# rageworx/libsrcnn

Hardware: AMD Instinct MI355X
Metric: megapixels/sec SRCNN Y-channel (2x upscale) (higher is better)
Workload: dtype f32

## Files before the change

### libsrcnn_amd/build.py

```python
import os
import subprocess
import sys

HERE = os.path.dirname(os.path.abspath(__file__))
CSRC = os.path.join(HERE, "csrc")
LIBDIR = os.path.join(HERE, "lib")
LIB = os.path.join(LIBDIR, "libsrcnn_amd.so")

SOURCES = ["srcnn_kernels.hip", "srcnn_fused_f16.hip", "srcnn_yuv_planes.hip", "srcnn_yuv_packed.hip", "srcnn_rgb.hip", "srcnn_rgb_window.hip", "srcnn_yuv_window.hip", "srcnn_yuv_packed_window.hip", "srcnn_window.hip", "srcnn_capi.cpp", "srcnn_frames.cpp", "srcnn_pipeline.cpp", "srcnn_comm.cpp", "dropin.cpp"]
DEPS = SOURCES + ["../../tools/srcnntest.cpp", "../../tools/srcnnyuv.cpp", "srcnn_kernels.h", "srcnn_yuv.h", "srcnn_rgb.h", "srcnn_window.h", "srcnn_frame_rules.h", "srcnn_frame_args.hpp", "srcnn_rect_source.hpp", "srcnn_pixel_io.h", "srcnn_colour_rules.h", "srcnn_window_tile.h", "srcnn_yuv_packed_fields.h", "srcnn_host.hpp", "srcnn_owned.hpp", "srcnn_settings.hpp", "srcnn_watchdog.hpp", "resample_table.hpp", "srcnn_weights.inc",
                  "../../include/srcnn_amd.h", "../../include/srcnn_amd_debug.h", "../../include/srcnn_amd_yuv.h", "../../include/srcnn_amd_yuv_ex.h", "../../include/srcnn_amd_yuv_packed.h", "../../include/srcnn_amd_rgb.h", "../../include/srcnn_amd_rect.h", "../../include/srcnn_amd_rgb_rect.h", "../../include/srcnn_amd_yuv_rect.h", "../../include/srcnn_amd_yuv_packed_rect.h",
                  "../../include/libsrcnn_dropin.h", "exports.map"]

FLAGS = ["--offload-arch=gfx950", "-O3", "-ffp-contract=off", "-fPIC", "-std=c++17",
         "-fvisibility=hidden", "-Wall", "-Wno-unused-result", "-Wno-unused-value", "-Wno-ignored-attributes", "-D__HIP_PLATFORM_AMD__"]


EXTRA_FLAGS = {"srcnn_fused_f16.hip": ["-fno-slp-vectorize"] + os.environ.get("SRCNN_FUSED_CFLAGS", "").split()}


def hipcc():
    for c in (os.environ.get("HIPCC"), "/opt/rocm/bin/hipcc", "hipcc"):
        if c and (os.path.isabs(c) and os.path.exists(c) or not os.path.isabs(c)):
            return c
    return "hipcc"


STAMP = os.path.join(LIBDIR, "build.sha256")


def source_digest():
    import hashlib
    h = hashlib.sha256()
    h.update(repr((FLAGS, sorted(EXTRA_FLAGS.items()))).encode())
    for d in sorted(set(DEPS)) + [os.path.abspath(__file__)]:
        path = d if os.path.isabs(d) else os.path.join(CSRC, d)
        h.update(os.path.basename(path).encode() + b"\0")
        with open(path, "rb") as f:
            h.update(f.read())
    return h.hexdigest()


def stale():
    if not all(os.path.exists(p) for p in (LIB, STAMP, os.path.join(LIBDIR, "libsrcnn.so"), os.path.join(LIBDIR, "libsrcnn.a"))):
        return True
    try:
        return open(STAMP).read().strip() != source_digest()
    except OSError:
        return True


def _region(src, start_pat, end_pat):
    import re
    m = re.search(start_pat, src)
    if not m:
        return None
    e = re.search(end_pat, src[m.end():])
    return src[m.start():m.end() + (e.start() if e else len(src) - m.end())]


def kernel_source_sha(name="k_conv12_mfma"):
    import hashlib
    import re
    src = open(os.path.join(CSRC, "srcnn_kernels.hip")).read()
    m = re.search(r"template <[^>]*>\s*__global__[^\n]*void %s\(" % re.escape(name), src)
    if not m:
        return None
    end = src.find("// ====", m.end())
    parts = [src[m.start():end if end > 0 else len(src)]]
    extra = []
    if name == "k_conv12_mfma":
        extra = [_region(src, r"constexpr int M_NW\b", r"\n// One tap-step"),
                 _region(src, r"__device__ __forceinline__ void rs_dma_dword\(", r"\n}\n"),
                 _region(src, r"void conv12_grid_info\(", r"\n}\n"),
                 _region(src, r"void launch_conv12_mfma\(", r"\n}\n"),
                 _region(open(os.path.join(CSRC, "srcnn_capi.cpp")).read(), r"void run_conv12\(", r"\n}\n")]
    elif name == "k_conv3":
        extra = [_region(src, r"constexpr int C3_TW\b", r"\ntemplate <bool STRICT"),
                 _region(src, r"__device__ __forceinline__ void rs_dma_dword\(", r"\n}\n"),
                 _region(src, r"void launch_conv3\(", r"\n}\n")]
    if any(e is None for e in extra):
        return None
    h = hashlib.sha256()
    for part in parts + extra:
        h.update(part.encode())
        h.update(b"\0")
    return h.hexdigest()


STRICT_DIR = os.path.join(LIBDIR, "strict")
STRICT_LIB = os.path.join(STRICT_DIR, "libsrcnn_amd.so")


def build_strict_only(force=False, verbose=True):
    import time
    stamp = os.path.join(STRICT_DIR, "build.sha256")
    digest = source_digest() + "-strict"
    if not force and os.path.exists(STRICT_LIB) and os.path.exists(stamp) and open(stamp).read().strip() == digest:
        return STRICT_LIB, None
    os.makedirs(STRICT_DIR, exist_ok=True)
    t0 = time.time()
    objs = []
    for src in SOURCES:
        if src == "srcnn_fused_f16.hip":
            continue
        obj = os.path.join(STRICT_DIR, os.path.splitext(src)[0] + ".o")
        cmd = [hipcc()] + FLAGS + ["-DSRCNN_STRICT_ONLY"] + ["-x", "hip", "-c", os.path.join(CSRC, src), "-o", obj]
        if verbose:
            print(" ".join(cmd), flush=True)
        subprocess.check_call(cmd)
        objs.append(obj)
    cmd = [hipcc(), "--offload-arch=gfx950", "-shared", "-fPIC"] + objs + ["-o", STRICT_LIB, "-ldl", "-Wl,-soname,libsrcnn_amd.so",
                                                                          "-Wl,--version-script=" + os.path.join(CSRC, "exports.map")]
    if verbose:
        print(" ".join(cmd), flush=True)
    subprocess.check_call(cmd)
    with open(stamp, "w") as f:
        f.write(digest + "\n")
    return STRICT_LIB, time.time() - t0


def build(force=False, verbose=True):
    if not force and not stale():
        return LIB
    os.makedirs(LIBDIR, exist_ok=True)
    objs = []
    for src in SOURCES:
        obj = os.path.join(LIBDIR, os.path.splitext(src)[0] + ".o")
        cmd = [hipcc()] + FLAGS + EXTRA_FLAGS.get(src, []) + ["-x", "hip", "-c", os.path.join(CSRC, src), "-o", obj]
        if verbose:
            print(" ".join(cmd), flush=True)
        subprocess.check_call(cmd)
# ... 38 lines not shown
```

### libsrcnn_amd/csrc/srcnn_capi.cpp

```cpp
#include <dlfcn.h>
#include <hip/hip_runtime.h>
#include <sys/prctl.h>
#include <sys/syscall.h>
#include <unistd.h>

#include <algorithm>
#include <cstdio>
#include <cstdlib>
#include <cstring>
#include <string>
#include <thread>

#include "resample_table.hpp"
#include <chrono>
#include <sys/auxv.h>
#include <unistd.h>

#include "../../include/srcnn_amd_rect.h"
#include "srcnn_frame_args.hpp"
#include "srcnn_host.hpp"
#include "srcnn_rect_source.hpp"
#include "srcnn_window.h"

namespace srcnn {
// ... 823 lines not shown
                        unsigned r0, unsigned r1, float* d_dst)
{
    return resample_src_rows(c, YSource::from_plane(d_in), sw, sh, dw, dh, filter, r0, r1, d_dst);
}

int check_plane(const void* in, unsigned w, unsigned h, const void* out)
{
    if (!in || !out || w == 0 || h == 0) return fail(SRCNN_E_ARG, "NULL pointer or zero dimension");
    if ((unsigned long long)w * h > 0x7fffffffULL) return fail(SRCNN_E_UNSUPPORTED, "plane too large");
    return SRCNN_OK;
}

int y_path_rows(Call& c, const YSource& src, unsigned w, unsigned h, unsigned dw, unsigned dh, int filter,
                unsigned r0, unsigned r1, float* d_out)
{
    if (r1 > dh || r0 >= r1) return fail(SRCNN_E_ARG, "row range [%u,%u) outside 0..%u", r0, r1, dh);
    if (dh > (1u << 20) || h > (1u << 20) || dw > 0x7fffffu || (r1 - r0) > 65535u * 16u)
        return fail(SRCNN_E_UNSUPPORTED, "output %ux%u too large", dw, dh);
    Workspace& ws = *c.ws;
    [[maybe_unused]] Ctx& cx = *c.cx;
    const unsigned ca = r0 >= 2 ? r0 - 2 : 0, cb = std::min(dh, r1 + 2);
    const unsigned ua = ca >= 4 ? ca - 4 : 0, ub = std::min(dh, cb + 4);
    int rc;
    if ((rc = ws.grow(ws.up, (size_t)dw * (ub - ua)))) return rc;
#ifndef SRCNN_STRICT_ONLY
    const bool fused = c.mode == SRCNN_MODE_FAST_F16;
    if (fused) {
        {
            StageTimer t(SRCNN_STAGE_RESAMPLE, c);
            if ((rc = resample_src_rows(c, src, w, h, dw, dh, filter, ua, ub, ws.up.data()))) return rc;
        }
        {
            StageTimer t(SRCNN_STAGE_CONV12, c);
            launch_fused_f16(ws.up.data(), (int)dw, (int)dh, (int)ua, (int)(ub - ua), d_out, (int)r0, (int)(r1 - r0), cx.fused_w.data(),
                             cx.num_cus, c.s);
        }
        HIP_TRY(hipGetLastError());
        return SRCNN_OK;
    }
#endif
    if ((rc = ws.grow(ws.c2, (size_t)C2N * dw * (cb - ca)))) return rc;
    TraceRange tr("srcnn y_path rows [%u,%u) of %ux%u", r0, r1, dw, dh);
    {
        StageTimer t(SRCNN_STAGE_RESAMPLE, c);
        if ((rc = resample_src_rows(c, src, w, h, dw, dh, filter, ua, ub, ws.up.data()))) return rc;
    }
    const size_t plane = (size_t)dw * (cb - ca);
    {
        StageTimer t(SRCNN_STAGE_CONV12, c);
        run_conv12(c, ws.up.data(), (int)dw, (int)dh, (int)ua, (int)(ub - ua), ws.c2.data(), plane, (int)ca, (int)(cb - ca));
    }
    {
        StageTimer t(SRCNN_STAGE_CONV3, c);
        launch_conv3(ws.c2.data(), plane, (int)dw, (int)dh, (int)ca, (int)(cb - ca), d_out, (int)r0, (int)(r1 - r0),
                     c.relax(), c.s);
    }
    if (const hipError_t e = hipGetLastError(); e != hipSuccess) {
        ws.queue_dirty = true;
        return fail(SRCNN_E_HIP, "y_path_rows: %s", hipGetErrorString(e));
    }
    return SRCNN_OK;
}

int y_path_source_rows(Call& c, unsigned h, unsigned dh, int filter, unsigned r0, unsigned r1, unsigned& lo, unsigned& hi)
{
    const unsigned ca = r0 >= 2 ? r0 - 2 : 0, cb = std::min(dh, r1 + 2);
    const unsigned ua = ca >= 4 ? ca - 4 : 0, ub = std::min(dh, cb + 4);
    if (h == dh) { lo = ua; hi = ub; return SRCNN_OK; }
    TableRef tv;
    int rc = get_table(c, filter, dh, h, tv);
    if (rc) return rc;
    tv->source_span(ua, ub, lo, hi);
    hi = std::min(hi, h);
    return SRCNN_OK;
}

unsigned budget_band_rows(unsigned dw)
{
    const size_t budget = G.ws_budget.load();
    const size_t row_bytes = (size_t)C2N * dw * sizeof(float);
    const size_t fit = budget / row_bytes;
    return (unsigned)std::min<size_t>(std::max<size_t>(16, fit > 4 ? fit - 4 : 1), 1u << 20);
}

std::vector<unsigned> plan_cuts(unsigned R0, unsigned R1, unsigned dw, unsigned dh, const double* frac, int nfrac, int grid, int tile_rows)
{
    const unsigned rows = R1 - R0;
    std::vector<unsigned> cuts{R0};
    const unsigned tiles_x = (dw + 63) / 64;
    unsigned a = R0;
    for (int i = 0; i < nfrac; ++i) {
        const unsigned want = std::max(32u, (unsigned)(rows * frac[i]));
        unsigned b = a + (want & ~15u);
        if (grid > 0 && tile_rows > 0) {
            const unsigned top = a >= 2 ? 2 : a;
            const unsigned t_want = (want + top + 2 + tile_rows - 1) / tile_rows;
            const unsigned t_lo = std::max(1u, (unsigned)(t_want * 0.7)), t_hi = std::max(t_lo, (unsigned)(t_want * 1.3));
            double best = -1.0;
            unsigned best_t = t_want;
            for (unsigned t = t_lo; t <= t_hi; ++t) {
                const unsigned long long tiles = (unsigned long long)t * tiles_x;
                const unsigned long long rounds = (tiles + grid - 1) / grid;
                const double fill = (double)tiles / (double)(rounds * grid);
                const double score = fill - 1e-4 * (t > t_want ? t - t_want : t_want - t);
                if (score > best) { best = score; best_t = t; }
            }
            if (best_t * tile_rows > top + 2) b = a + best_t * tile_rows - top - 2;
// ... 25 lines not shown
}

int y_path_frame(Call& c, const float* d_in, unsigned w, unsigned h, unsigned dw, unsigned dh, int filter, float* d_out)
{
    return y_path_range(c, d_in, w, h, dw, dh, filter, 0, dh, d_out);
}

namespace {

int y_path_rect_rows(Call& c, const float* d_in, size_t in_stride, unsigned in_x0, unsigned in_y0, unsigned w, unsigned h,
                     unsigned dw, unsigned dh, int filter, unsigned x0, unsigned x1, unsigned r0, unsigned r1, float* d_out,
                     size_t out_stride)
{
    Workspace& ws = *c.ws;
    [[maybe_unused]] Ctx& cx = *c.cx;
    const unsigned cax = x0 >= 2 ? x0 - 2 : 0, cbx = std::min(dw, x1 + 2);
    const unsigned uax = cax >= 4 ? cax - 4 : 0, ubx = std::min(dw, cbx + 4);
    const unsigned Ww = ubx - uax;
    const unsigned ca = r0 >= 2 ? r0 - 2 : 0, cb = std::min(dh, r1 + 2);
    const unsigned ua = ca >= 4 ? ca - 4 : 0, ub = std::min(dh, cb + 4);
    int rc;
    if ((rc = ws.grow(ws.up, (size_t)Ww * (ub - ua)))) return rc;
    if ((rc = ws.grow(ws.win, (size_t)Ww * (r1 - r0)))) return rc;
    const float* interior = ws.win.data() + (x0 - uax);
#ifndef SRCNN_STRICT_ONLY
    if (c.mode == SRCNN_MODE_FAST_F16) {
        {
            StageTimer t(SRCNN_STAGE_RESAMPLE, c);
            if ((rc = resample_window(c, d_in, in_stride, in_x0, in_y0, w, h, dw, dh, filter, uax, ubx, ua, ub, ws.up.data()))) return rc;
        }
        {
            StageTimer t(SRCNN_STAGE_CONV12, c);
            launch_fused_f16(ws.up.data(), (int)Ww, (int)dh, (int)ua, (int)(ub - ua), ws.win.data(), (int)r0, (int)(r1 - r0), cx.fused_w.data(),
                             cx.num_cus, c.s);
        }
        launch_window_copy(interior, Ww, d_out, out_stride, (int)(x1 - x0), (int)(r1 - r0), c.s);
        HIP_TRY(hipGetLastError());
        return SRCNN_OK;
    }
#endif
    if ((rc = ws.grow(ws.c2, (size_t)C2N * Ww * (cb - ca)))) return rc;
    TraceRange tr("srcnn y_path rect [%u,%u)x[%u,%u) of %ux%u", x0, x1, r0, r1, dw, dh);
    {
        StageTimer t(SRCNN_STAGE_RESAMPLE, c);
        if ((rc = resample_window(c, d_in, in_stride, in_x0, in_y0, w, h, dw, dh, filter, uax, ubx, ua, ub, ws.up.data()))) return rc;
    }
    const size_t plane = (size_t)Ww * (cb - ca);
    {
        StageTimer t(SRCNN_STAGE_CONV12, c);
        run_conv12(c, ws.up.data(), (int)Ww, (int)dh, (int)ua, (int)(ub - ua), ws.c2.data(), plane, (int)ca, (int)(cb - ca));
    }
    {
        StageTimer t(SRCNN_STAGE_CONV3, c);
        launch_conv3(ws.c2.data(), plane, (int)Ww, (int)dh, (int)ca, (int)(cb - ca), ws.win.data(), (int)r0, (int)(r1 - r0), c.relax(), c.s);
    }
    launch_window_copy(interior, Ww, d_out, out_stride, (int)(x1 - x0), (int)(r1 - r0), c.s);
    if (const hipError_t e = hipGetLastError(); e != hipSuccess) {
        ws.queue_dirty = true;
        return fail(SRCNN_E_HIP, "y_path_rect: %s", hipGetErrorString(e));
    }
    return SRCNN_OK;
}

}

int y_path_rect(Call& c, const float* d_in, size_t in_stride, unsigned in_x0, unsigned in_y0, unsigned w, unsigned h, unsigned dw,
                unsigned dh, int filter, unsigned x0, unsigned y0, unsigned x1, unsigned y1, float* d_out, size_t out_stride, bool whole_plane)
{
    if (x1 > dw || x0 >= x1 || y1 > dh || y0 >= y1) return fail(SRCNN_E_ARG, "rect [%u,%u)x[%u,%u) outside %ux%u", x0, x1, y0, y1, dw, dh);
    if (dh > (1u << 20) || h > (1u << 20) || dw > 0x7fffffu || (y1 - y0) > 65535u * 16u)
        return fail(SRCNN_E_UNSUPPORTED, "output %ux%u too large", dw, dh);
    if (x0 == 0 && x1 == dw && whole_plane && in_x0 == 0 && in_y0 == 0 && in_stride == w && out_stride == dw)
        return y_path_range(c, d_in, w, h, dw, dh, filter, y0, y1, d_out);
    const unsigned cax = x0 >= 2 ? x0 - 2 : 0, cbx = std::min(dw, x1 + 2);
    const unsigned Ww = std::min(dw, cbx + 4) - (cax >= 4 ? cax - 4 : 0);
    const size_t row_bytes = (size_t)C2N * Ww * sizeof(float);
    const bool no_planes = c.mode == SRCNN_MODE_FAST_F16;
    if (no_planes || row_bytes * ((size_t)(y1 - y0) + 4) <= G.ws_budget.load())
        return y_path_rect_rows(c, d_in, in_stride, in_x0, in_y0, w, h, dw, dh, filter, x0, x1, y0, y1, d_out, out_stride);
    const unsigned band = budget_band_rows(Ww);
    for (unsigned a = y0; a < y1; a += band) {
        const unsigned b = std::min(y1, a + band);
        int rc = y_path_rect_rows(c, d_in, in_stride, in_x0, in_y0, w, h, dw, dh, filter, x0, x1, a, b, d_out + (size_t)(a - y0) * out_stride, out_stride);
        if (rc) return rc;
    }
    return SRCNN_OK;
}

unsigned y_path_rect_band_rows(const Call& c, unsigned dw, unsigned x0, unsigned x1, unsigned y0, unsigned y1)
{
    const unsigned cax = x0 >= 2 ? x0 - 2 : 0, cbx = std::min(dw, x1 + 2);
    const unsigned Ww = std::min(dw, cbx + 4) - (cax >= 4 ? cax - 4 : 0);
    const size_t row_bytes = (size_t)C2N * Ww * sizeof(float);
    if (c.mode == SRCNN_MODE_FAST_F16 || row_bytes * ((size_t)(y1 - y0) + 4) <= G.ws_budget.load()) return y1 - y0;
    return std::min(y1 - y0, budget_band_rows(Ww));
}

int check_y_path_args(const float* d_in, unsigned w, unsigned h, unsigned dw, unsigned dh, int filter, const float* d_out)
{
    int rc = check_plane(d_in, w, h, d_out);
    if (rc) return rc;
    if (dw == 0 || dh == 0) return fail(SRCNN_E_SCALE, "scaled size %ux%u", dw, dh);
    if (filter < 0 || filter > 4) return fail(SRCNN_E_ARG, "bad filter %d", filter);
    return SRCNN_OK;
}

namespace {
// ... 518 lines not shown
    {
        std::lock_guard<std::mutex> lk(cx->mu);
        drain_spans_locked(*cx);
        if (total_ms) *total_ms = cx->stage_ms[stage];
        if (launches) *launches = cx->stage_n[stage];
    }
    if (Ctx* cur = context_at(srcnn_get_context())) (void)hipSetDevice(cur->device);
    return SRCNN_OK;
}

int srcnn_resample_f32_dev(const float* d_in, unsigned w, unsigned h, unsigned dw, unsigned dh, int filter,
                           float* d_out, void* stream)
{
    int rc;
    if ((rc = check_y_path_args(d_in, w, h, dw, dh, filter, d_out))) return rc;
    if (dh > (1u << 20) || h > (1u << 20)) return fail(SRCNN_E_UNSUPPORTED, "too many rows");
    StreamCall sc(stream);
    if (sc.rc) return sc.rc;
    rc = resample_rows_range(sc.c, d_in, w, h, dw, dh, filter, 0, dh, d_out);
    if (rc) return rc;
    HIP_TRY(hipGetLastError());
    return SRCNN_OK;
}

int srcnn_conv1_f32_dev(const float* d_y, unsigned w, unsigned h, float* d_c1, void* stream)
{
    int rc;
    if ((rc = check_plane(d_y, w, h, d_c1))) return rc;
    if (h > 65535u * 4u) return fail(SRCNN_E_UNSUPPORTED, "too many rows");
    if (!ctx_for_stream(stream)) return SRCNN_E_NODEVICE;
    launch_conv1_planes(d_y, (int)w, (int)h, d_c1, (hipStream_t)stream);
    HIP_TRY(hipGetLastError());
    return SRCNN_OK;
}

int srcnn_conv2_f32_dev(const float* d_c1, unsigned w, unsigned h, float* d_c2, void* stream)
{
    int rc;
    if ((rc = check_plane(d_c1, w, h, d_c2))) return rc;
    if (!ctx_for_stream(stream)) return SRCNN_E_NODEVICE;
    launch_conv2_planes(d_c1, (size_t)w * h, d_c2, (hipStream_t)stream);
    HIP_TRY(hipGetLastError());
    return SRCNN_OK;
}

int srcnn_conv3_f32_dev(const float* d_c2, unsigned w, unsigned h, float* d_out, void* stream)
{
    int rc;
    if ((rc = check_plane(d_c2, w, h, d_out))) return rc;
    if (h > 65535u * 16u) return fail(SRCNN_E_UNSUPPORTED, "too many rows");
    if (!ctx_for_stream(stream)) return SRCNN_E_NODEVICE;
    Call c;
    c.mode = G.mode.load();
    launch_conv3(d_c2, (size_t)w * h, (int)w, (int)h, 0, (int)h, d_out, 0, (int)h, c.relax(), (hipStream_t)stream);
    HIP_TRY(hipGetLastError());
    return SRCNN_OK;
}

int srcnn_conv12_f32_dev(const float* d_y, unsigned w, unsigned h, float* d_c2, void* stream)
{
    int rc;
    if ((rc = check_plane(d_y, w, h, d_c2))) return rc;
    if (h > 65535u * 4u) return fail(SRCNN_E_UNSUPPORTED, "too many rows");
    Call c;
    c.cx = ctx_for_stream(stream);
    if (!c.cx) return SRCNN_E_NODEVICE;
    c.s = (hipStream_t)stream; c.mode = G.mode.load();
    run_conv12(c, d_y, (int)w, (int)h, 0, (int)h, d_c2, (size_t)w * h, 0, (int)h);
    HIP_TRY(hipGetLastError());
    return SRCNN_OK;
}

int srcnn_axis_table(int filter, unsigned dst_len, unsigned src_len, int* left, int* right, double* weights)
{
    if (dst_len == 0 || src_len == 0) return fail(SRCNN_E_ARG, "zero length");
    const srcnn::AxisTable t = srcnn::build_axis_table(filter, dst_len, src_len);
    if (left) memcpy(left, t.first.data(), sizeof(int) * dst_len);
    if (right) memcpy(right, t.last.data(), sizeof(int) * dst_len);
    if (weights) memcpy(weights, t.weight.data(), sizeof(double) * t.weight.size());
    return t.window;
}

int srcnn_fused_diag(const float* d_up, unsigned w, unsigned h, float* d_out, unsigned long long* d_dbg, void* stream)
{
    int rc;
    if ((rc = check_plane(d_up, w, h, d_out))) return rc;
#ifdef SRCNN_STRICT_ONLY
    (void)d_dbg; (void)stream;
    return fail(SRCNN_E_UNSUPPORTED, "strict-only build: the fused fp16 kernel is not compiled in");
#else
    Ctx* cx = ctx_for_stream(stream);
    if (!cx) return SRCNN_E_NODEVICE;
    launch_fused_f16(d_up, (int)w, (int)h, 0, (int)h, d_out, 0, (int)h, cx->fused_w.data(), cx->num_cus, (hipStream_t)stream, d_dbg);
    HIP_TRY(hipGetLastError());
    return SRCNN_OK;
#endif
}

int srcnn_debug_settings(char* buf, size_t cap, int markdown)
{
    const std::string t = settings().describe(markdown != 0);
    if (buf && cap) snprintf(buf, cap, "%s", t.c_str());
    return (int)t.size();
}

int srcnn_debug_counts(int* tables, int* lanes)
{
// ... 14 lines not shown
```

### libsrcnn_amd/csrc/srcnn_kernels.h

```cpp
#pragma once
#include <hip/hip_runtime.h>
#include <stddef.h>

namespace srcnn {

constexpr int C1N = 64;
constexpr int C2N = 32;
enum : int {
    RELAX_L1 = 1,
    RELAX_L2 = 2,
    RELAX_L3_X64 = 4,
    RELAX_L3_F32 = 8,
    RELAX_FAST = RELAX_L1 | RELAX_L2 | RELAX_L3_F32
};
constexpr int kWeightCount = 64 + 64 * 81 + 32 + 32 * 64 + 1 + 32 * 25;

struct DevWeights {
    float w1t[81][C1N];
    float b1[C1N];
    float w2[C2N][C1N];
    float b2[C2N];
    float w3[C2N][25];
    float b3;
    float pad_[3];
// ... 9 lines not shown
    int monotone;
    const int* h_first;
    const int* h_taps;
};

struct YSource {
    const float* plane = nullptr;
    const unsigned char* rgb = nullptr;
    int depth = 0;
    static YSource from_plane(const float* p) { YSource y; y.plane = p; return y; }
    static YSource from_rgb(const unsigned char* p, int d) { YSource y; y.rgb = p; y.depth = d; return y; }
};

#ifndef FU_NW_DEF
#define FU_NW_DEF 8
#endif
constexpr int FU_NK = 5;
constexpr int FU_NW = FU_NW_DEF;
struct FusedF16Weights {
    unsigned short w1[FU_NK][2][2][64][8];
    unsigned short w2[2][2][2][64][8];
    unsigned short w3[2][2][64][8];
    float b1[64];
    float b2[32];
    float w88[64];
    float b3;
    float pad_[3];
};

hipError_t upload_weights(const DevWeights& w);
hipError_t fused_f16_prepare();
void launch_fused_f16(const float* Y, int W, int H, int y_row_base, int y_rows, float* out, int out_row0, int out_rows,
                      const FusedF16Weights* d_blob, int num_cus, hipStream_t s, unsigned long long* dbg = nullptr);

void launch_resample_cols(const float* src, int w, int src_row_base, float* dst, int dst_row0, int dst_rows,
                          const DevAxisTable& t, hipStream_t s);
void launch_resample_rows(const float* src, int src_w, float* dst, int dst_w, int rows, const DevAxisTable& t,
                          hipStream_t s);
bool launch_rs2d(const YSource& src, int src_w, int src_h, float* dst, int dst_w, int dst_h, int dst_row0, int dst_rows,
                 const DevAxisTable& tv, const DevAxisTable& th, hipStream_t s);
hipError_t rs2d_prepare();
bool rs2d_fits(int np, int src_w, int src_h, int dst_w, int dst_h, int r0, int r1, const DevAxisTable& tv, const DevAxisTable& th);
bool launch_merge_fused(const unsigned char* rgb_src, int src_w, int src_h, int depth, const float* Yp,
                        unsigned char* rgb_out, unsigned char* conv_opt, int dst_w, int dst_h, int dst_row0, int dst_rows,
                        const DevAxisTable& tv, const DevAxisTable& th, hipStream_t s);
hipError_t conv12_mfma_prepare();
void launch_conv12_mfma(const float* Y, int W, int H, int y_row_base, int y_rows, float* C2, size_t plane_stride, int out_row0,
                        int out_rows, int relax, int num_cus, hipStream_t s, unsigned long long* clk = nullptr,
                        unsigned* queue = nullptr);
void conv12_grid_info(int num_cus, int* blocks, int* tile_rows);
constexpr int kConv12TileRows = 16, kConv12BlocksPerCU = 2;
void launch_conv3(const float* C2, size_t plane_stride, int W, int H, int c2_row_base, int c2_rows, float* out,
                  int out_row0, int out_rows, int relax, hipStream_t s);
void launch_conv1_planes(const float* Y, int W, int H, float* C1, hipStream_t s);
void launch_conv2_planes(const float* C1, size_t n, float* C2v, hipStream_t s);
void launch_rgb_split(const unsigned char* rgb, size_t n, int d, float* Yp, float* Cb, float* Cr, float* A,
                      hipStream_t s);
void launch_ycc_merge(const float* Yp, const float* Cb, const float* Cr, const float* A, size_t n, int d,
                      unsigned char* rgb, unsigned char* conv_opt, hipStream_t s);

}
```

### libsrcnn_amd/csrc/srcnn_kernels.hip

```cpp
#include <hip/hip_runtime.h>
#include <type_traits>
#include <stdint.h>
#include <stdlib.h>
#include <algorithm>
#include "srcnn_kernels.h"
#include "srcnn_settings.hpp"

#pragma clang fp contract(off)

namespace srcnn {

__constant__ DevWeights cW;

hipError_t upload_weights(const DevWeights& w)
{
    return hipMemcpyToSymbol(HIP_SYMBOL(cW), &w, sizeof(DevWeights));
}

__device__ __forceinline__ int clampi(int v, int lo, int hi) { return v < lo ? lo : (v > hi ? hi : v); }

__global__ __launch_bounds__(256) void k_resample_cols(
    const float* __restrict__ src, int w, int src_row_base,
    float* __restrict__ dst, int dst_row0, int dst_rows,
    const int* __restrict__ first, const int* __restrict__ taps, const double* __restrict__ wt, int stride)
// ... 1036 lines not shown
    float sum[4][2] = {};
    issue(0);
    land(tile[0]);
    __syncthreads();
#pragma unroll 1
    for (int c = 0; c < C2N / CF_MC; ++c) {
        const float* cur = tile[c & 1];
        if (c + 1 < C2N / CF_MC) issue((c + 1) * CF_MC);
#pragma unroll 1
        for (int m = 0; m < CF_MC; ++m) {
            const float* t = cur + m * CF_CH + (wv * 4) * CF_LW + 2 * lane;
            const float* wm = cW.w3[c * CF_MC + m];
            float win[8][6];
#pragma unroll
            for (int r = 0; r < 8; ++r)
#pragma unroll
                for (int p = 0; p < 3; ++p) {
                    const float2 v = *reinterpret_cast<const float2*>(t + r * CF_LW + 2 * p);
                    win[r][2 * p] = v.x; win[r][2 * p + 1] = v.y;
                }
            float a[4][2] = {};
#pragma unroll
            for (int dy = 0; dy < 5; ++dy)
#pragma unroll
                for (int dx = 0; dx < 5; ++dx) {
                    const float wgt = wm[dy * 5 + dx];
#pragma unroll
                    for (int q = 0; q < 4; ++q) {
                        a[q][0] = __builtin_fmaf(wgt, win[q + dy][dx], a[q][0]);
                        a[q][1] = __builtin_fmaf(wgt, win[q + dy][dx + 1], a[q][1]);
                    }
                }
#pragma unroll
            for (int q = 0; q < 4; ++q) { sum[q][0] += a[q][0]; sum[q][1] += a[q][1]; }
        }
        if (c + 1 < C2N / CF_MC) land(tile[(c + 1) & 1]);
        __syncthreads();
    }
#pragma unroll
    for (int q = 0; q < 4; ++q) {
        const int row = ty0 + wv * 4 + q;
        if (row < H && row < out_row0 + out_rows) {
#pragma unroll
            for (int e = 0; e < 2; ++e) {
                const int x = tx0 + 2 * lane + e;
                if (x < W) out[(size_t)(row - out_row0) * W + x] = fminf(fmaxf(sum[q][e] + cW.b3, 0.f), 255.f);
            }
        }
    }
}

#endif

__global__ __launch_bounds__(256) void k_conv1_planes(const float* __restrict__ Y, int W, int H,
                                                      float* __restrict__ C1, size_t plane_stride)
{
    const int x = blockIdx.x * 64 + (threadIdx.x & 63);
    const int y = blockIdx.y * 4 + (threadIdx.x >> 6);
    const int k0 = blockIdx.z * 8;
    if (x >= W || y >= H) return;
    float acc[8] = {0, 0, 0, 0, 0, 0, 0, 0};
    for (int i = 0; i < 9; ++i) {
        const int gy = clampi(y + i - 4, 0, H - 1);
        for (int j = 0; j < 9; ++j) {
            const float v = Y[(size_t)gy * W + clampi(x + j - 4, 0, W - 1)];
#pragma unroll
            for (int k = 0; k < 8; ++k) acc[k] = acc[k] + cW.w1t[i * 9 + j][k0 + k] * v;
        }
    }
#pragma unroll
    for (int k = 0; k < 8; ++k)
        C1[(size_t)(k0 + k) * plane_stride + (size_t)y * W + x] = fmaxf(acc[k] + cW.b1[k0 + k], 0.f);
}

__global__ __launch_bounds__(256) void k_conv2_planes(const float* __restrict__ C1, size_t n,
                                                      float* __restrict__ C2v)
{
    const size_t p = (size_t)blockIdx.x * 256 + threadIdx.x;
    const int m0 = blockIdx.y * 8;
    if (p >= n) return;
    float acc[8] = {0, 0, 0, 0, 0, 0, 0, 0};
    for (int f = 0; f < C1N; ++f) {
        const float v = C1[(size_t)f * n + p];
#pragma unroll
        for (int m = 0; m < 8; ++m) acc[m] = acc[m] + v * cW.w2[m0 + m][f];
    }
#pragma unroll
    for (int m = 0; m < 8; ++m) C2v[(size_t)(m0 + m) * n + p] = fmaxf(acc[m] + cW.b2[m0 + m], 0.f);
}

__global__ __launch_bounds__(256) void k_rgb_split(const unsigned char* __restrict__ rgb, size_t n, int d,
                                                   float* __restrict__ Yp, float* __restrict__ Cb,
                                                   float* __restrict__ Cr, float* __restrict__ A)
{
    const size_t p = (size_t)blockIdx.x * 256 + threadIdx.x;
    if (p >= n) return;
    const float r = (float)rgb[p * d + 0], g = (float)rgb[p * d + 1], b = (float)rgb[p * d + 2];
    Yp[p] = (0.299f * r) + (0.587f * g) + (0.114f * b);
    Cb[p] = 128.f - (0.1687f * r) - (0.3313f * g) + (0.5f * b);
    Cr[p] = 128.f + (0.5f * r) - (0.4187f * g) - (0.0813f * b);
    if (d == 4) A[p] = (float)rgb[p * d + 3];
}

__global__ __launch_bounds__(256) void k_ycc_merge(const float* __restrict__ Yp, const float* __restrict__ Cb,
                                                   const float* __restrict__ Cr, const float* __restrict__ A,
                                                   size_t n, int d, unsigned char* __restrict__ rgb,
// ... 195 lines not shown
#ifdef SRCNN_STRICT_ONLY
    (void)relax;
    if (settings().conv12_dma) CONV12_GO(0, true); else CONV12_GO(0, false);
#else
    switch (relax & 3) {
    case 0: if (settings().conv12_dma) CONV12_GO(0, true); else CONV12_GO(0, false); break;
    case 1: CONV12_GO(1, true); break;
    case 2: CONV12_GO(2, true); break;
    default: CONV12_GO(3, true); break;
    }
#endif
#undef CONV12_GO
}

void launch_conv3(const float* C2, size_t plane_stride, int W, int H, int c2_row_base, int c2_rows, float* out,
                  int out_row0, int out_rows, int relax, hipStream_t s)
{
    if (out_rows <= 0) return;
#ifndef SRCNN_STRICT_ONLY
    const bool strict = !(relax & (RELAX_L3_X64 | RELAX_L3_F32));
    const bool wide_planes = (size_t)c2_rows * (size_t)W * sizeof(float) >= ((size_t)1 << 32);
    if (relax & RELAX_L3_X64) {
        const dim3 gx(cdiv(W, 64), cdiv(out_rows, 16));
        if (wide_planes)
            hipLaunchKernelGGL((k_conv3<true, true, true>), gx, dim3(256), 0, s, C2, plane_stride, W, H, c2_row_base, c2_rows, out, out_row0, out_rows, 0);
        else
            hipLaunchKernelGGL((k_conv3<true, false, true>), gx, dim3(256), 0, s, C2, plane_stride, W, H, c2_row_base, c2_rows, out, out_row0, out_rows, 0);
        return;
    }
    if (!strict) {
        dim3 gridf(cdiv(W, CF_TW), cdiv(out_rows, CF_TH));
        hipLaunchKernelGGL(k_conv3_fast, gridf, dim3(256), 0, s, C2, plane_stride, W, H, c2_row_base, c2_rows, out,
                           out_row0, out_rows);
        return;
    }
#else
    (void)relax;
#endif
    dim3 grid(cdiv(W, 64), cdiv(out_rows, 16));
    const bool force_wide = settings().conv3_off64;
    const int wdma = settings().conv3_wdma ? 1 : 0;
    const bool wide = force_wide || (size_t)c2_rows * (size_t)W * sizeof(float) >= ((size_t)1 << 32);
    if (!wide && wdma)
        hipLaunchKernelGGL((k_conv3<true, false, false, true>), grid, dim3(256), 0, s, C2, plane_stride, W, H, c2_row_base, c2_rows,
                           out, out_row0, out_rows, 1);
    else if (!wide)
        hipLaunchKernelGGL((k_conv3<true, false>), grid, dim3(256), 0, s, C2, plane_stride, W, H, c2_row_base, c2_rows,
                           out, out_row0, out_rows, wdma);
    else
        hipLaunchKernelGGL((k_conv3<true, true>), grid, dim3(256), 0, s, C2, plane_stride, W, H, c2_row_base, c2_rows,
                           out, out_row0, out_rows, wdma);
}

void launch_conv1_planes(const float* Y, int W, int H, float* C1, hipStream_t s)
{
    dim3 grid(cdiv(W, 64), cdiv(H, 4), C1N / 8);
    hipLaunchKernelGGL(k_conv1_planes, grid, dim3(256), 0, s, Y, W, H, C1, (size_t)W * H);
}

void launch_conv2_planes(const float* C1, size_t n, float* C2v, hipStream_t s)
{
    dim3 grid((unsigned)((n + 255) / 256), C2N / 8);
    hipLaunchKernelGGL(k_conv2_planes, grid, dim3(256), 0, s, C1, n, C2v);
}

template <int D>
__global__ __launch_bounds__(256) void k_rgb_split4(const unsigned* __restrict__ rgb32, size_t n4,
                                                    float4* __restrict__ Yp, float4* __restrict__ Cb,
                                                    float4* __restrict__ Cr, float4* __restrict__ A)
{
    const size_t q = (size_t)blockIdx.x * 256 + threadIdx.x;
    if (q >= n4) return;
    unsigned wds[D];
#pragma unroll
    for (int k = 0; k < D; ++k) wds[k] = rgb32[q * D + k];
    float yv[4], cbv[4], crv[4], av[4];
#pragma unroll
    for (int i = 0; i < 4; ++i) {
        float ch[4] = {0.f, 0.f, 0.f, 0.f};
#pragma unroll
        for (int k = 0; k < D; ++k) {
            const int byte = i * D + k;
            ch[k] = (float)((wds[byte >> 2] >> (8 * (byte & 3))) & 0xffu);
        }
        const float r = ch[0], g = ch[1], b = ch[2];
        yv[i] = (0.299f * r) + (0.587f * g) + (0.114f * b);
        cbv[i] = 128.f - (0.1687f * r) - (0.3313f * g) + (0.5f * b);
        crv[i] = 128.f + (0.5f * r) - (0.4187f * g) - (0.0813f * b);
        av[i] = ch[3];
    }
    Yp[q] = make_float4(yv[0], yv[1], yv[2], yv[3]);
    Cb[q] = make_float4(cbv[0], cbv[1], cbv[2], cbv[3]);
    Cr[q] = make_float4(crv[0], crv[1], crv[2], crv[3]);
    if (D == 4) A[q] = make_float4(av[0], av[1], av[2], av[3]);
}

template <int D, bool CONV>
__global__ __launch_bounds__(256) void k_ycc_merge4(const float4* __restrict__ Yp, const float4* __restrict__ Cb,
                                                    const float4* __restrict__ Cr, const float4* __restrict__ A,
                                                    size_t n4, unsigned* __restrict__ rgb32, unsigned* __restrict__ conv32)
{
    const size_t q = (size_t)blockIdx.x * 256 + threadIdx.x;
    if (q >= n4) return;
    const float4 y4 = Yp[q], cb4 = Cb[q], cr4 = Cr[q];
    float4 a4 = make_float4(0.f, 0.f, 0.f, 0.f);
    if (D == 4) a4 = A[q];
// ... 78 lines not shown
```

### libsrcnn_amd/csrc/srcnn_settings.hpp

```cpp
#pragma once
#include <cstddef>
#include <string>

#define SRCNN_SETTINGS(X)                                                                                                          \
                                                                                                            \
    X(S, devices,          "SRCNN_DEVICES",          "",    "unset = device 0, `all`, `0,1,...`", "contexts of a process that never calls `srcnn_init*` (an id may repeat: virtual contexts on one device)") \
    X(I, max_workspace_mb, "SRCNN_MAX_WORKSPACE_MB", 4608, "MiB (API twin `srcnn_set_workspace_limit`)", "layer-2 scratch one pass may hold; larger ranges are banded, bit-identically.  The default holds a whole 7680x4320 output frame (4.25 GB); lower it where memory is short: 2048 costs -1...+2 % by box, 512 +2 %, 256 +9 % (`profiles/r06_lowmem.txt`); 16384 until round 6") \
    X(I, max_lanes,        "SRCNN_MAX_LANES",        4,     "1...64", "concurrent `ProcessSRCNN` calls per context before callers queue") \
    X(B, numa,             "SRCNN_NUMA",             1,     "0/1", "place page-locked staging on the device's NUMA node (the caller's memory policy is saved and restored)") \
    X(I, comm_timeout_ms,  "SRCNN_COMM_TIMEOUT_MS",  60000, "ms, 0 = none (API twin `srcnn_comm_set_timeout_ms`)", "deadline of every wait on a peer") \
    X(B, comm_check,       "SRCNN_COMM_CHECK",       1,     "0/1", "all-reduce a checksum of every new gather table across the ranks before the first gather that uses it") \
    X(S, rccl_lib,         "SRCNN_RCCL_LIB",         "",    "path", "load this RCCL instead of the one next to the bound `libamdhip64` (site builds; the test-suite's one-device stand-in).  A trust boundary: the named file's code runs in the process; refused under secure execution (`AT_SECURE`)") \
    X(I, async_chain,      "SRCNN_ASYNC_CHAIN",      1,     "0/1/2", "order the kernels of consecutive asynchronous `ProcessSRCNN` jobs: 0 = not at all, 1 = on the host, 2 = with device-side event waits") \
    X(B, trace,            "SRCNN_TRACE",            0,     "0/1", "one stderr line per `srcnn_process_u8` share (setup / bands / stamps)") \
    X(B, roctx,            "SRCNN_ROCTX",            0,     "0/1", "roctx ranges for `rocprofv3 --marker-trace`") \
    X(S, bands,            "SRCNN_BANDS",            "",    "`f0,f1,...`", "band fractions of a large `ProcessSRCNN` image instead of the planned cuts") \
    X(I, graph_max_cpu_pct, "SRCNN_GRAPH_MAX_CPU_PCT", 10,  "0...100, 0 = never fall back", "`srcnn_y_upscale2x_f32_stream(use_graph = 1)`: hipGraph replay is kept only while the process's CPU time per replayed frame stays below this share of the frame's wall time (plain launches cost 6-8 % of a 4K frame; replay on ROCm 7.2 costs 20 % in a fresh process and ~100 % -- a runtime thread spinning from launch to completion -- in a process with more streams); above it the stream goes on with plain launches: same kernels, same overlap") \
    X(B, prefault,         "SRCNN_PREFAULT",         1,     "0/1", "pre-fault the fresh result pages of `ProcessSRCNN` in the background") \
    X(I, prefault_threads, "SRCNN_PREFAULT_THREADS", 1,     ">= 1", "helpers of that pre-faulting") \
    X(B, thp,              "SRCNN_THP",              1,     "0/1", "huge-page hint on large result blocks") \
    X(B, spin_wait,        "SRCNN_SPIN_WAIT",        0,     "0/1", "host waits through the runtime (holds a core) instead of polling") \
    X(B, device_wait_in,   "SRCNN_DEVICE_WAIT_IN",   0,     "0/1", "bands wait for their stage-in device-side (a runtime thread stays busy)") \
                   \
    X(B, conv12_queue,     "SRCNN_CONV12_QUEUE",     1,     "0/1", "layer 1+2: tiles drawn from a global counter vs dealt with a static stride") \
    X(B, conv12_dma,       "SRCNN_CONV12_DMA",       1,     "0/1", "layer 1+2: weights and Y tiles staged by LDS-DMA one tile ahead vs load, wait, `ds_write`") \
    X(B, conv12_prune,     "SRCNN_CONV12_PRUNE",     1,     "0/1", "layer 1+2: strict layer 2 skips the 15 near-dead layer-1 channels in every 32-pixel segment where they are all zero vs always multiplies all 64") \
    X(B, conv12_spread,    "SRCNN_CONV12_SPREAD",    1,     "0/1", "layer 1+2: small launches dealt in quarter tiles over up to 4x more workgroups") \
    X(B, conv3_wdma,       "SRCNN_CONV3_WDMA",       1,     "0/1", "layer 3: packed weight image staged by LDS-DMA vs a plain loop") \
    X(B, conv3_off64,      "SRCNN_CONV3_OFF64",      0,     "0/1", "layer 3: 64-bit plane offsets (chosen automatically for planes of 4 GiB or more)") \
    X(B, rs_dma,           "SRCNN_RS_DMA",           1,     "0/1", "resampler: `k_rs2d_dma` (source patch by LDS-DMA) vs `k_rs2d` for plane sources") \
    X(I, rs_tpb,           "SRCNN_RS_TPB",           0,     "0 = auto, 1...16", "resampler: row tiles a block marches through") \
    X(B, resample_2pass,   "SRCNN_RESAMPLE_2PASS",   0,     "0/1", "resampler: always the two generic passes (`k_resample_cols/rows`, what down-scales use); implies the unfused colour shell") \
    X(B, shell_unfused,    "SRCNN_SHELL_UNFUSED",    0,     "0/1", "colour shell as split + plane resamples + merge instead of fused into the resampler") \
    X(B, rgb_rect_unfused, "SRCNN_RGB_RECT_UNFUSED", 0,     "0/1", "RGB(A) rect call: window unpack + window plane resamples + pack for every shape instead of `k_rgb_window_merge` for up-scales") \
    X(B, yuv_rect_unfused, "SRCNN_YUV_RECT_UNFUSED", 0,     "0/1", "YUV rect call: chroma by window unpack + window plane resamples + pack for every shape instead of `k_yuv_window_chroma` for up-scales") \
    X(B, yuv_packed_rect_unfused, "SRCNN_YUV_PACKED_RECT_UNFUSED", 0, "0/1", "packed YUV rect call: window unpack + window plane resamples + pack for every shape instead of `k_yuvp_window_merge` for up-scales")

namespace srcnn {

struct Settings {
#define SRCNN_SET_B(m, d) bool m = (d) != 0;
#define SRCNN_SET_I(m, d) long m = (d);
#define SRCNN_SET_S(m, d) std::string m = d;
#define X(kind, member, env, def, values, effect) SRCNN_SET_##kind(member, def)
    SRCNN_SETTINGS(X)
#undef X
#undef SRCNN_SET_B
#undef SRCNN_SET_I
#undef SRCNN_SET_S
    static Settings from_env();
    std::string describe(bool markdown) const;
};

const Settings& settings();

}
```

Before: 3726.

## Add sparse layer-3 kernel skipping all-zero layer-2 channel windows per wave

Adds k_conv3_sparse, a strict layer-3 convolution that, for four candidate layer-2 channels (1, 13, 26, 29), checks by wave ballot whether the activations just read into LDS are all zero over the wave's window and skips that channel's 5x5 multiply-accumulate if so. A new launch_layer3 dispatcher selects it by default in strict mode and otherwise falls back to launch_conv3. The work saved depends on how often those channels are exactly zero after ReLU. In exchange it adds a per-channel ballot check and duplicates the conv3 tile pipeline, with the weight DMA inlined.

```diff
diff --git a/libsrcnn_amd/build.py b/libsrcnn_amd/build.py
--- a/libsrcnn_amd/build.py
+++ b/libsrcnn_amd/build.py
@@ -64,9 +64,13 @@
     import re
     src = open(os.path.join(CSRC, "srcnn_kernels.hip")).read()
     m = re.search(r"template <[^>]*>\s*__global__[^\n]*void %s\(" % re.escape(name), src)
+    if not m and name == "k_conv3_sparse":
+        m = re.search(r"// =+\n// conv3, strict, skipping all-zero channel windows", src)
+        if m and not re.search(r"__global__[^\n]*void k_conv3_sparse\(", src[m.end():src.find("// ====", src.find("__global__", m.end()))]):
+            m = None
     if not m:
         return None
-    end = src.find("// ====", m.end())
+    end = src.find("// ====", src.find("__global__", m.end()) if name == "k_conv3_sparse" else m.end())
     parts = [src[m.start():end if end > 0 else len(src)]]
     extra = []
     if name == "k_conv12_mfma":
@@ -78,6 +82,11 @@
     elif name == "k_conv3":
         extra = [_region(src, r"constexpr int C3_TW\b", r"\ntemplate <bool STRICT"),
                  _region(src, r"__device__ __forceinline__ void rs_dma_dword\(", r"\n}\n"),
+                 _region(src, r"void launch_conv3\(", r"\n}\n")]
+    elif name == "k_conv3_sparse":
+        extra = [_region(src, r"constexpr int C3_TW\b", r"\ntemplate <bool STRICT"),
+                 _region(src, r"__device__ __forceinline__ void rs_dma_dword\(", r"\n}\n"),
+                 _region(src, r"void launch_layer3\(", r"\n}\n"),
                  _region(src, r"void launch_conv3\(", r"\n}\n")]
     if any(e is None for e in extra):
         return None
diff --git a/libsrcnn_amd/csrc/srcnn_capi.cpp b/libsrcnn_amd/csrc/srcnn_capi.cpp
--- a/libsrcnn_amd/csrc/srcnn_capi.cpp
+++ b/libsrcnn_amd/csrc/srcnn_capi.cpp
@@ -899,7 +899,7 @@
     }
     {
         StageTimer t(SRCNN_STAGE_CONV3, c);
-        launch_conv3(ws.c2.data(), plane, (int)dw, (int)dh, (int)ca, (int)(cb - ca), d_out, (int)r0, (int)(r1 - r0),
+        launch_layer3(ws.c2.data(), plane, (int)dw, (int)dh, (int)ca, (int)(cb - ca), d_out, (int)r0, (int)(r1 - r0),
                      c.relax(), c.s);
     }
     if (const hipError_t e = hipGetLastError(); e != hipSuccess) {
@@ -1031,7 +1031,7 @@
     }
     {
         StageTimer t(SRCNN_STAGE_CONV3, c);
-        launch_conv3(ws.c2.data(), plane, (int)Ww, (int)dh, (int)ca, (int)(cb - ca), ws.win.data(), (int)r0, (int)(r1 - r0), c.relax(), c.s);
+        launch_layer3(ws.c2.data(), plane, (int)Ww, (int)dh, (int)ca, (int)(cb - ca), ws.win.data(), (int)r0, (int)(r1 - r0), c.relax(), c.s);
     }
     launch_window_copy(interior, Ww, d_out, out_stride, (int)(x1 - x0), (int)(r1 - r0), c.s);
     if (const hipError_t e = hipGetLastError(); e != hipSuccess) {
@@ -1656,7 +1656,7 @@
     if (!ctx_for_stream(stream)) return SRCNN_E_NODEVICE;
     Call c;
     c.mode = G.mode.load();
-    launch_conv3(d_c2, (size_t)w * h, (int)w, (int)h, 0, (int)h, d_out, 0, (int)h, c.relax(), (hipStream_t)stream);
+    launch_layer3(d_c2, (size_t)w * h, (int)w, (int)h, 0, (int)h, d_out, 0, (int)h, c.relax(), (hipStream_t)stream);
     HIP_TRY(hipGetLastError());
     return SRCNN_OK;
 }
diff --git a/libsrcnn_amd/csrc/srcnn_kernels.h b/libsrcnn_amd/csrc/srcnn_kernels.h
--- a/libsrcnn_amd/csrc/srcnn_kernels.h
+++ b/libsrcnn_amd/csrc/srcnn_kernels.h
@@ -85,6 +85,8 @@
 constexpr int kConv12TileRows = 16, kConv12BlocksPerCU = 2;
 void launch_conv3(const float* C2, size_t plane_stride, int W, int H, int c2_row_base, int c2_rows, float* out,
                   int out_row0, int out_rows, int relax, hipStream_t s);
+void launch_layer3(const float* C2, size_t plane_stride, int W, int H, int c2_row_base, int c2_rows, float* out,
+                   int out_row0, int out_rows, int relax, hipStream_t s);
 void launch_conv1_planes(const float* Y, int W, int H, float* C1, hipStream_t s);
 void launch_conv2_planes(const float* C1, size_t n, float* C2v, hipStream_t s);
 void launch_rgb_split(const unsigned char* rgb, size_t n, int d, float* Yp, float* Cb, float* Cr, float* A,
diff --git a/libsrcnn_amd/csrc/srcnn_kernels.hip b/libsrcnn_amd/csrc/srcnn_kernels.hip
--- a/libsrcnn_amd/csrc/srcnn_kernels.hip
+++ b/libsrcnn_amd/csrc/srcnn_kernels.hip
@@ -1112,6 +1112,146 @@
 
 #endif
 
+constexpr unsigned C3_SPARSE = 0x24002002u;
+
+__global__ __launch_bounds__(256, 6) void k_conv3_sparse(
+    const float* __restrict__ C2, size_t plane_stride, int W, int H, int c2_row_base, int c2_rows,
+    float* __restrict__ out, int out_row0, int out_rows)
+{
+    constexpr int C3_MC = c3_mc(true);
+    __shared__ float tile[2][C3_MC * C3_CH];
+    __shared__ __attribute__((aligned(16))) float w3s[C2N * 30];
+
+    const int tx0 = blockIdx.x * C3_TW;
+    const int ty0 = out_row0 + blockIdx.y * C3_TH;
+    const int tid = threadIdx.x, lane = tid & 63, wv = tid >> 6;
+    const int c2_last = c2_row_base + c2_rows - 1;
+    const int wave_e0 = __builtin_amdgcn_readfirstlane(tid & ~63);
+#pragma unroll
+    for (int i = 0; i < (C2N * 30 + 255) / 256; ++i) {
+        const int e = tid + i * 256;
+        if (e < C2N * 30) rs_dma_dword(cW.w3p + e, w3s + i * 256 + wave_e0);
+    }
+
+    const int bx = min(tx0 + lane, W - 1);
+    const int hq = tid & 3;
+    const int hx = clampi(tx0 + (hq < 2 ? hq - 2 : 62 + hq), 0, W - 1);
+    const int hlc = hq < 2 ? hq : 64 + hq;
+    auto row_of = [&](int r) {
+        int gy = clampi(ty0 + r - 2, 0, H - 1);
+        gy = clampi(gy, c2_row_base, c2_last);
+        return gy - c2_row_base;
+    };
+    unsigned boff[C3_LH / 4];
+#pragma unroll
+    for (int j = 0; j < C3_LH / 4; ++j) boff[j] = ((unsigned)row_of(4 * j + wv) * (unsigned)W + (unsigned)bx) * 4u;
+    const int wv_s = __builtin_amdgcn_readfirstlane(wv);
+    float halo4[C3_MC];
+    const int h4row = min(tid >> 2, C3_LH - 1);
+    const unsigned h4off = ((unsigned)row_of(h4row) * (unsigned)W + (unsigned)hx) * 4u;
+    auto issue_dma = [&](int mc, float* dst) {
+        if (tid < C3_LH * 4) {
+#pragma unroll
+            for (int m = 0; m < C3_MC; ++m)
+                halo4[m] = *reinterpret_cast<const float*>(reinterpret_cast<const char*>(C2 + (size_t)(mc + m) * plane_stride) + h4off);
+        }
+#pragma unroll
+        for (int m = 0; m < C3_MC; ++m) {
+            const unsigned long long pb = reinterpret_cast<unsigned long long>(C2 + (size_t)(mc + m) * plane_stride);
+            const unsigned ub_hi = (unsigned)__builtin_amdgcn_readfirstlane((int)(unsigned)(pb >> 32));
+            const unsigned ub_lo = (unsigned)__builtin_amdgcn_readfirstlane((int)(unsigned)pb);
+            const unsigned long long ub = ((unsigned long long)ub_hi << 32) | (unsigned long long)ub_lo;
+#pragma unroll
+            for (int j = 0; j < C3_LH / 4; ++j)
+                rs_dma_dword_s(reinterpret_cast<const void*>(ub), boff[j], dst + (wv_s + 4 * (m * (C3_LH / 4) + j)) * C3_LW + 2);
+        }
+    };
+    auto land_dma = [&](float* dst) {
+        if (tid < C3_LH * 4) {
+#pragma unroll
+            for (int m = 0; m < C3_MC; ++m) dst[m * C3_CH + h4row * C3_LW + hlc] = halo4[m];
+        }
+        asm volatile("s_waitcnt vmcnt(0)" ::: "memory");
+    };
+
+    float sum[4] = {0.f, 0.f, 0.f, 0.f};
+    issue_dma(0, tile[0]);
+    land_dma(tile[0]);
+    asm volatile("s_waitcnt vmcnt(0)" ::: "memory");
+    __syncthreads();
+
+    const int offA = (wv * 4) * C3_LW + lane;
+    int offB = offA + 4 * C3_LW;
+    asm volatile("" : "+v"(offB));
+
+#pragma unroll 1
+    for (int c = 0; c < C2N / C3_MC; ++c) {
+        const float* cur = tile[c & 1];
+        if (c + 1 < C2N / C3_MC) issue_dma((c + 1) * C3_MC, tile[(c + 1) & 1]);
+#pragma unroll 1
+        for (int m = 0; m < C3_MC; ++m) {
+            typedef float f2 __attribute__((ext_vector_type(2)));
+            const float* tA = cur + m * C3_CH + offA;
+            const float* tB = cur + m * C3_CH + offB;
+            f2 va[8], vb[8], vp[7];
+#pragma unroll
+            for (int r = 0; r < 4; ++r) {
+                va[r] = f2{tA[r * C3_LW + 0], tA[r * C3_LW + 1]};
+                vb[r] = f2{tA[r * C3_LW + 2], tA[r * C3_LW + 3]};
+                va[r + 4] = f2{tB[r * C3_LW + 0], tB[r * C3_LW + 1]};
+                vb[r + 4] = f2{tB[r * C3_LW + 2], tB[r * C3_LW + 3]};
+            }
+#pragma unroll
+            for (int k = 0; k < 3; ++k) {
+                vp[k] = f2{tA[k * C3_LW + 4], tA[(k + 1) * C3_LW + 4]};
+                vp[k + 4] = f2{tB[k * C3_LW + 4], tB[(k + 1) * C3_LW + 4]};
+            }
+            vp[3] = f2{tA[3 * C3_LW + 4], tB[4]};
+            if ((C3_SPARSE >> (c * C3_MC + m)) & 1u) {
+                unsigned bits = 0;
+#pragma unroll
+                for (int r = 0; r < 8; ++r) bits |= __float_as_uint(va[r].x);
+#pragma unroll
+                for (int k = 0; k < 8; k += 2) bits |= __float_as_uint(vp[k].x) | __float_as_uint(vp[k].y);
+                if (__builtin_amdgcn_ballot_w64((bits & 0x7fffffffu) != 0u) == 0ull) continue;
+            }
+            const float* wrow = w3s + (c * C3_MC + m) * 30;
+            double a[4] = {0.0, 0.0, 0.0, 0.0};
+#pragma unroll
+            for (int dy = 0; dy < 5; ++dy) {
+                const f2 wa = f2{wrow[dy * 6 + 0], wrow[dy * 6 + 1]};
+                const f2 wb = f2{wrow[dy * 6 + 2], wrow[dy * 6 + 3]};
+                const f2 wc = f2{wrow[dy * 6 + 4], wrow[dy * 6 + 4]};
+                const f2 pc01 = wc * vp[dy], pc23 = wc * vp[dy + 2];
+#pragma unroll
+                for (int q = 0; q < 4; ++q) {
+                    const f2 pa = wa * va[q + dy], pb = wb * vb[q + dy];
+                    const float pc = q == 0 ? pc01.x : q == 1 ? pc01.y : q == 2 ? pc23.x : pc23.y;
+                    a[q] = (dy == 0) ? (double)pa.x : a[q] + (double)pa.x;
+                    a[q] = a[q] + (double)pa.y;
+                    a[q] = a[q] + (double)pb.x;
+                    a[q] = a[q] + (double)pb.y;
+                    a[q] = a[q] + (double)pc;
+                }
+            }
+#pragma unroll
+            for (int q = 0; q < 4; ++q) sum[q] = (float)((double)sum[q] + a[q]);
+        }
+        if (c + 1 < C2N / C3_MC) land_dma(tile[(c + 1) & 1]);
+        __syncthreads();
+    }
+    const int x = tx0 + lane;
+#pragma unroll
+    for (int q = 0; q < 4; ++q) {
+        const int row = ty0 + wv * 4 + q;
+        if (x < W && row < H && row < out_row0 + out_rows) {
+            float v = sum[q] + cW.b3;
+            v = fminf(fmaxf(v, 0.f), 255.f);
+            out[(size_t)(row - out_row0) * W + x] = v;
+        }
+    }
+}
+
 __global__ __launch_bounds__(256) void k_conv1_planes(const float* __restrict__ Y, int W, int H,
                                                       float* __restrict__ C1, size_t plane_stride)
 {
@@ -1413,6 +1553,24 @@
                            out, out_row0, out_rows, wdma);
 }
 
+void launch_layer3(const float* C2, size_t plane_stride, int W, int H, int c2_row_base, int c2_rows, float* out,
+                   int out_row0, int out_rows, int relax, hipStream_t s)
+{
+    if (out_rows <= 0) return;
+#ifndef SRCNN_STRICT_ONLY
+    const bool strict = !(relax & (RELAX_L3_X64 | RELAX_L3_F32));
+#else
+    const bool strict = true;
+#endif
+    const bool wide = settings().conv3_off64 || (size_t)c2_rows * (size_t)W * sizeof(float) >= ((size_t)1 << 32);
+    if (strict && !wide && settings().conv3_wdma && settings().conv3_skip) {
+        hipLaunchKernelGGL(k_conv3_sparse, dim3(cdiv(W, C3_TW), cdiv(out_rows, C3_TH)), dim3(256), 0, s, C2, plane_stride, W, H,
+                           c2_row_base, c2_rows, out, out_row0, out_rows);
+        return;
+    }
+    launch_conv3(C2, plane_stride, W, H, c2_row_base, c2_rows, out, out_row0, out_rows, relax, s);
+}
+
 void launch_conv1_planes(const float* Y, int W, int H, float* C1, hipStream_t s)
 {
     dim3 grid(cdiv(W, 64), cdiv(H, 4), C1N / 8);
diff --git a/libsrcnn_amd/csrc/srcnn_settings.hpp b/libsrcnn_amd/csrc/srcnn_settings.hpp
--- a/libsrcnn_amd/csrc/srcnn_settings.hpp
+++ b/libsrcnn_amd/csrc/srcnn_settings.hpp
@@ -28,6 +28,7 @@
     X(B, conv12_spread,    "SRCNN_CONV12_SPREAD",    1,     "0/1", "layer 1+2: small launches dealt in quarter tiles over up to 4x more workgroups") \
     X(B, conv3_wdma,       "SRCNN_CONV3_WDMA",       1,     "0/1", "layer 3: packed weight image staged by LDS-DMA vs a plain loop") \
     X(B, conv3_off64,      "SRCNN_CONV3_OFF64",      0,     "0/1", "layer 3: 64-bit plane offsets (chosen automatically for planes of 4 GiB or more)") \
+    X(B, conv3_skip,       "SRCNN_CONV3_SKIP",       1,     "0/1", "layer 3: `k_conv3_sparse`, where a wave skips a layer-2 channel of the candidate set {1, 13, 26, 29} whose activations it has just read as all zero over its 68x8 window, vs `k_conv3`, which always runs all 32") \
     X(B, rs_dma,           "SRCNN_RS_DMA",           1,     "0/1", "resampler: `k_rs2d_dma` (source patch by LDS-DMA) vs `k_rs2d` for plane sources") \
     X(I, rs_tpb,           "SRCNN_RS_TPB",           0,     "0 = auto, 1...16", "resampler: row tiles a block marches through") \
     X(B, resample_2pass,   "SRCNN_RESAMPLE_2PASS",   0,     "0/1", "resampler: always the two generic passes (`k_resample_cols/rows`, what down-scales use); implies the unfused colour shell") \
```

Result: faster. 3768 (median of 6 runs) (+1.1%).
